# ActiveVisionLab/CrossScore

Measured on AMD Instinct MI355X. Metric: query-images/sec at 518x518, 5 ref views, bs=8; score-map MAE vs ref, higher is better.
Workload: dtype fp16

## Files before the change

### crossscore_amd/csrc/rowln.hip

```cpp
#include "cs_common.h"
#include <atomic>

namespace {

__device__ __forceinline__ float rl_add_other_half(float x) {
  const auto r = __builtin_amdgcn_permlane32_swap(__float_as_uint(x), __float_as_uint(x), false, false);
  return __uint_as_float(r[0]) + __uint_as_float(r[1]);
}

template <int C, bool BF, int G2>
__global__ __launch_bounds__(C / 96 * 64) void cs_rowln_kernel(CsRowLnParams p) {
  constexpr int NW = C / 96, NT = NW * 64;
  constexpr bool NEXT = G2 > 0;
  constexpr int BK = 64, NSL = C / BK;
  constexpr int APITCH = C * 2 + 16;
  constexpr int WPITCH = BK * 2 + 16;
  constexpr int WBUF = C * WPITCH;
  constexpr int ACH = C / 8, WCH = BK / 8;
  constexpr int AIT = 64 * ACH / NT, WIT = C * WCH / NT;
  static_assert(64 * ACH % NT == 0 && C * WCH % NT == 0, "staging maps");
  extern __shared__ __attribute__((aligned(16))) char smem[];
  char* As = smem;
  char* Ws = smem + 64 * APITCH;
  float* red = reinterpret_cast<float*>(Ws + 2 * WBUF);
  const int tid = threadIdx.x;
  const int lane = tid & 63;
  const int wv = __builtin_amdgcn_readfirstlane(tid >> 6);
  const int j = lane & 31, h = lane >> 5;
  const int row0 = blockIdx.x * 64;
  const int col0 = wv * 96;
  uint4 wreg[WIT];
#define RL_LOAD_W(REG, WP, LDW, SL)                                                                                \
  _Pragma("unroll") for (int it = 0; it < WIT; ++it) {                                                         \
    const int c_ = tid + it * NT, r_ = c_ / WCH, ch_ = c_ - r_ * WCH;                                          \
    REG[it] = *reinterpret_cast<const uint4*>((WP) + (size_t)r_ * (LDW) + (SL) * BK + ch_ * 8);                \
  }
#define RL_WRITE_W(REG, BUF)                                                                                   \
  _Pragma("unroll") for (int it = 0; it < WIT; ++it) {                                                         \
    const int c_ = tid + it * NT, r_ = c_ / WCH, ch_ = c_ - r_ * WCH;                                          \
    *reinterpret_cast<uint4*>(Ws + (BUF) * WBUF + r_ * WPITCH + ch_ * 16) = REG[it];                           \
  }
  RL_LOAD_W(wreg, p.W, p.ldw, 0)
  {
    uint4 areg[AIT];
#pragma unroll
    for (int it = 0; it < AIT; ++it) {
      const int c = tid + it * NT, r = c / ACH, ch = c - r * ACH;
      areg[it] = *reinterpret_cast<const uint4*>(p.A + (size_t)min(row0 + r, p.M - 1) * p.lda + ch * 8);
    }
#pragma unroll
    for (int it = 0; it < AIT; ++it) {
      const int c = tid + it * NT, r = c / ACH, ch = c - r * ACH;
      *reinterpret_cast<uint4*>(As + r * APITCH + ch * 16) = areg[it];
    }
  }
#define RL_KSLICE(SLICE)                                                                                       \
  _Pragma("unroll") for (int ks = 0; ks < BK / 16; ++ks) {                                                     \
    h16x8_t a[2], w[3];                                                                                        \
    _Pragma("unroll") for (int rb = 0; rb < 2; ++rb)                                                           \
      a[rb] = *reinterpret_cast<const h16x8_t*>(a_rd + rb * 32 * APITCH + ((SLICE) * (BK / 16) + ks) * 32);    \
    _Pragma("unroll") for (int ct = 0; ct < 3; ++ct) w[ct] = *reinterpret_cast<const h16x8_t*>(w_rd + ct * 32 * WPITCH + ks * 32); \
    _Pragma("unroll") for (int rb = 0; rb < 2; ++rb)                                                           \
      _Pragma("unroll") for (int ct = 0; ct < 3; ++ct) acc[rb][ct] = mfma_32x32x16<BF>(w[ct], a[rb], acc[rb][ct]); \
  }
  RL_WRITE_W(wreg, 0)
  __syncthreads();
  f32x16_t acc[2][3];
#pragma unroll
  for (int rb = 0; rb < 2; ++rb)
#pragma unroll
    for (int ct = 0; ct < 3; ++ct)
#pragma unroll
      for (int e = 0; e < 16; ++e) acc[rb][ct][e] = 0.f;
  const char* a_rd = As + j * APITCH + h * 16;
  for (int sl = 0; sl < NSL; ++sl) {
    if (sl + 1 < NSL) { RL_LOAD_W(wreg, p.W, p.ldw, sl + 1) }
    const char* w_rd = Ws + (sl & 1) * WBUF + (col0 + j) * WPITCH + h * 16;
    RL_KSLICE(sl)
    if (sl + 1 < NSL) { RL_WRITE_W(wreg, (sl + 1) & 1) }
    __syncthreads();
  }
  f32x4_t gam[3][4], bet[3][4];
#pragma unroll
  for (int ct = 0; ct < 3; ++ct)
#pragma unroll
    for (int g = 0; g < 4; ++g) {
      const int c = col0 + 32 * ct + 8 * g + 4 * h;
      const f32x4_t b4 = *reinterpret_cast<const f32x4_t*>(p.bias + c);
      gam[ct][g] = *reinterpret_cast<const f32x4_t*>(p.gamma + c);
      bet[ct][g] = *reinterpret_cast<const f32x4_t*>(p.beta + c);
#pragma unroll
      for (int rb = 0; rb < 2; ++rb)
#pragma unroll
        for (int i = 0; i < 4; ++i) acc[rb][ct][4 * g + i] += b4[i];
    }
  if (p.resid) {
#pragma unroll
    for (int rb = 0; rb < 2; ++rb) {
      const float* rr = p.resid + (size_t)min(row0 + 32 * rb + j, p.M - 1) * p.ldr + col0 + 4 * h;
#pragma unroll
      for (int ct = 0; ct < 3; ++ct)
#pragma unroll
        for (int g = 0; g < 4; ++g) {
          const f32x4_t r4 = *reinterpret_cast<const f32x4_t*>(rr + 32 * ct + 8 * g);
#pragma unroll
          for (int i = 0; i < 4; ++i) acc[rb][ct][4 * g + i] += r4[i];
        }
    }
  }
  float mean[2], rstd[2];
#pragma unroll
  for (int rb = 0; rb < 2; ++rb) {
    float s = 0.f;
#pragma unroll
    for (int ct = 0; ct < 3; ++ct)
#pragma unroll
      for (int e = 0; e < 16; e += 4) s += (acc[rb][ct][e] + acc[rb][ct][e + 1]) + (acc[rb][ct][e + 2] + acc[rb][ct][e + 3]);
    s = rl_add_other_half(s);
    if (h == 0) red[(0 * NW + wv) * 64 + 32 * rb + j] = s;
  }
  __syncthreads();
#pragma unroll
  for (int rb = 0; rb < 2; ++rb) {
    float s = 0.f;
#pragma unroll
    for (int w2 = 0; w2 < NW; ++w2) s += red[(0 * NW + w2) * 64 + 32 * rb + j];
    mean[rb] = s * (1.0f / C);
    float q = 0.f;
#pragma unroll
    for (int ct = 0; ct < 3; ++ct)
#pragma unroll
      for (int e = 0; e < 16; ++e) {
        const float d = acc[rb][ct][e] - mean[rb];
        q = fmaf(d, d, q);
      }
    q = rl_add_other_half(q);
    if (h == 0) red[(1 * NW + wv) * 64 + 32 * rb + j] = q;
  }
  __syncthreads();
#pragma unroll
  for (int rb = 0; rb < 2; ++rb) {
    float q = 0.f;
#pragma unroll
    for (int w2 = 0; w2 < NW; ++w2) q += red[(1 * NW + w2) * 64 + 32 * rb + j];
    rstd[rb] = 1.0f / sqrtf(q * (1.0f / C) + p.eps);
  }
#pragma unroll
  for (int rb = 0; rb < 2; ++rb) {
    const int row = row0 + 32 * rb + j;
    if (row < p.M) {
      float* o32 = p.out_f32 ? p.out_f32 + (size_t)row * C + col0 + 4 * h : nullptr;
      h16_t* o16 = p.out_f16 ? p.out_f16 + (size_t)row * C + col0 + 4 * h : nullptr;
#pragma unroll
      for (int ct = 0; ct < 3; ++ct)
#pragma unroll
        for (int g = 0; g < 4; ++g) {
          f32x4_t y;
#pragma unroll
          for (int i = 0; i < 4; ++i) y[i] = (acc[rb][ct][4 * g + i] - mean[rb]) * rstd[rb] * gam[ct][g][i] + bet[ct][g][i];
          if (o32) *reinterpret_cast<f32x4_t*>(o32 + 32 * ct + 8 * g) = y;
          if (o16) {
            uint2 o;
            o.x = pack_o16x2<BF>(y[0], y[1]);
            o.y = pack_o16x2<BF>(y[2], y[3]);
            *reinterpret_cast<uint2*>(o16 + 32 * ct + 8 * g) = o;
          }
        }
    }
  }
  if constexpr (NEXT) {
#pragma unroll
    for (int rb = 0; rb < 2; ++rb) {
      char* arow = As + (32 * rb + j) * APITCH + (col0 + 4 * h) * 2;
#pragma unroll
      for (int ct = 0; ct < 3; ++ct)
#pragma unroll
        for (int g = 0; g < 4; ++g) {
          float y[4];
#pragma unroll
          for (int i = 0; i < 4; ++i) y[i] = (acc[rb][ct][4 * g + i] - mean[rb]) * rstd[rb] * gam[ct][g][i] + bet[ct][g][i];
          uint2 o;
          o.x = pack_o16x2<BF>(y[0], y[1]);
          o.y = pack_o16x2<BF>(y[2], y[3]);
          *reinterpret_cast<uint2*>(arow + (32 * ct + 8 * g) * 2) = o;
        }
    }
    RL_LOAD_W(wreg, p.W2, p.ldw2, 0)
    RL_WRITE_W(wreg, 0)
    __syncthreads();
    constexpr int nsl2 = G2 * NSL;
#pragma unroll
    for (int s2 = 0; s2 < nsl2; ++s2) {
      const int grp = s2 / NSL, sl = s2 - grp * NSL;
      if (sl == 0) {
#pragma unroll
        for (int rb = 0; rb < 2; ++rb)
#pragma unroll
          for (int ct = 0; ct < 3; ++ct)
#pragma unroll
            for (int e = 0; e < 16; ++e) acc[rb][ct][e] = 0.f;
      }
      if (s2 + 1 < nsl2) {
        const int g2 = (s2 + 1) / NSL, sn = (s2 + 1) - g2 * NSL;
        RL_LOAD_W(wreg, p.W2 + (size_t)g2 * C * p.ldw2, p.ldw2, sn)
      }
      const char* w_rd = Ws + (s2 & 1) * WBUF + (col0 + j) * WPITCH + h * 16;
      RL_KSLICE(sl)
      if (s2 + 1 < nsl2) { RL_WRITE_W(wreg, (s2 + 1) & 1) }
      __syncthreads();
      if (sl == NSL - 1) {
#pragma unroll
        for (int rb = 0; rb < 2; ++rb) {
          const int row = row0 + 32 * rb + j;
          if (row < p.M) {
            h16_t* o2 = p.out2 + (size_t)row * p.ld2 + grp * C + col0 + 4 * h;
            const float* b2 = p.bias2 + grp * C + col0 + 4 * h;
#pragma unroll
            for (int ct = 0; ct < 3; ++ct)
#pragma unroll
              for (int g = 0; g < 4; ++g) {
                const f32x4_t b4 = *reinterpret_cast<const f32x4_t*>(b2 + 32 * ct + 8 * g);
                float v[4];
#pragma unroll
                for (int i = 0; i < 4; ++i) {
                  v[i] = acc[rb][ct][4 * g + i] + b4[i];
                  if (p.act2 == 1) v[i] = fmaxf(v[i], 0.f);
                  if (p.act2 == 2) v[i] = v[i] >= 0.f ? v[i] : 0.01f * v[i];
                }
                uint2 o;
                o.x = pack_o16x2<BF>(v[0], v[1]);
                o.y = pack_o16x2<BF>(v[2], v[3]);
                *reinterpret_cast<uint2*>(o2 + 32 * ct + 8 * g) = o;
              }
          }
        }
      }
    }
  }
#undef RL_KSLICE
#undef RL_LOAD_W
#undef RL_WRITE_W
}

}

extern "C" int cs_rowln_supported(int C) { return C == 384; }

extern "C" const char* cs_rowln_check(const CsRowLnParams* p, int C) {
  if (!cs_rowln_supported(C)) return "linear + LayerNorm: built for C = 384";
  if (!p->A || !p->W || !p->bias || !p->gamma || !p->beta || (!p->out_f32 && !p->out_f16 && !p->n2)) return "linear + LayerNorm: null operand";
  if (p->n2) {
    if ((p->n2 != C && p->n2 != 3 * C) || p->act2 < 0 || p->act2 > 2) return "linear + LayerNorm: the second stage takes C or 3 C output columns and act2 in 0..2";
    if (!p->W2 || !p->bias2 || !p->out2) return "linear + LayerNorm: null operand (second stage)";
    if (p->ldw2 % 8 || p->ldw2 < C || p->ld2 % 4 || p->ld2 < p->n2) return "linear + LayerNorm: row strides must keep 16-byte rows (second stage)";
    if (((uintptr_t)p->W2 | (uintptr_t)p->bias2) & 15 || ((uintptr_t)p->out2 & 7)) return "linear + LayerNorm: operands must be 16-byte aligned (second stage)";
  }
  if (p->M <= 0) return "linear + LayerNorm: empty shape";
  if (p->lda % 8 || p->ldw % 8 || p->lda < C || p->ldw < C || (p->resid && (p->ldr % 4 || p->ldr < C))) return "linear + LayerNorm: row strides must keep 16-byte rows";
  if (((uintptr_t)p->A | (uintptr_t)p->W | (uintptr_t)p->bias | (uintptr_t)p->gamma | (uintptr_t)p->beta | (uintptr_t)p->resid | (uintptr_t)p->out_f32 |
       (uintptr_t)p->out_f16) & 15)
    return "linear + LayerNorm: operands must be 16-byte aligned";
  return nullptr;
}

extern "C" hipError_t cs_rowln_launch(const CsRowLnParams* p, int C, int bf16, hipStream_t st) {
  if (C != 384) return hipErrorInvalidValue;
  constexpr int CC = 384, NW = CC / 96;
  constexpr int lds = 64 * (CC * 2 + 16) + 2 * CC * (64 * 2 + 16) + 2 * NW * 64 * 4;
  static std::atomic<bool> attr_done[16];
  int dev = 0;
  if (hipGetDevice(&dev) != hipSuccess || dev < 0 || dev >= 16) return hipErrorInvalidDevice;
  if (!attr_done[dev]) {
    const void* fns[6] = {reinterpret_cast<const void*>(cs_rowln_kernel<384, true, 0>), reinterpret_cast<const void*>(cs_rowln_kernel<384, false, 0>),
                          reinterpret_cast<const void*>(cs_rowln_kernel<384, true, 1>), reinterpret_cast<const void*>(cs_rowln_kernel<384, false, 1>),
                          reinterpret_cast<const void*>(cs_rowln_kernel<384, true, 3>), reinterpret_cast<const void*>(cs_rowln_kernel<384, false, 3>)};
    for (const void* f : fns)
      if (hipError_t e = hipFuncSetAttribute(f, hipFuncAttributeMaxDynamicSharedMemorySize, lds); e != hipSuccess) return e;
    attr_done[dev] = true;
  }
  const dim3 grid((p->M + 63) / 64), block(NW * 64);
#define RL_GO(G) do { if (bf16) hipLaunchKernelGGL((cs_rowln_kernel<384, true, G>), grid, block, lds, st, *p);  \
                      else hipLaunchKernelGGL((cs_rowln_kernel<384, false, G>), grid, block, lds, st, *p); } while (0)
  if (p->n2 == 0) RL_GO(0);
  else if (p->n2 == CC) RL_GO(1);
  else if (p->n2 == 3 * CC) RL_GO(3);
  else return hipErrorInvalidValue;
#undef RL_GO
  return hipGetLastError();
}
```

Before: 1409.

## Split row-LN GEMM across 8 waves with 16x16 MFMA and unified weight pipeline

Doubles the block to 8 waves, splitting the 64 rows into two 32-row halves so each wave computes a 32x96 tile with 16x16x32 MFMAs instead of 64x96 with 32x32x16. The first GEMM and the follow-on GEMM groups are merged into one unrolled slice loop with two register buffers prefetching weights two slices ahead, which removes the separate W2 prologue stall. LayerNorm reductions now use permlane16+permlane32 swaps. The aim is more latency hiding and occupancy, at the cost of extra LDS traffic per MFMA and a larger unrolled code body.

```diff
diff --git a/crossscore_amd/csrc/rowln.hip b/crossscore_amd/csrc/rowln.hip
--- a/crossscore_amd/csrc/rowln.hip
+++ b/crossscore_amd/csrc/rowln.hip
@@ -3,21 +3,29 @@
 
 namespace {
 
-__device__ __forceinline__ float rl_add_other_half(float x) {
+typedef unsigned u32x4_t __attribute__((ext_vector_type(4)));
+
+__device__ __forceinline__ float rl_add_lane16(float x) {
+  const auto r = __builtin_amdgcn_permlane16_swap(__float_as_uint(x), __float_as_uint(x), false, false);
+  return __uint_as_float(r[0]) + __uint_as_float(r[1]);
+}
+__device__ __forceinline__ float rl_add_lane32(float x) {
   const auto r = __builtin_amdgcn_permlane32_swap(__float_as_uint(x), __float_as_uint(x), false, false);
   return __uint_as_float(r[0]) + __uint_as_float(r[1]);
 }
 
 template <int C, bool BF, int G2>
-__global__ __launch_bounds__(C / 96 * 64) void cs_rowln_kernel(CsRowLnParams p) {
-  constexpr int NW = C / 96, NT = NW * 64;
+__global__ __launch_bounds__(C / 96 * 128) void cs_rowln_kernel(CsRowLnParams p) {
+  constexpr int NW = C / 96, NT = NW * 128;
   constexpr bool NEXT = G2 > 0;
   constexpr int BK = 64, NSL = C / BK;
+  constexpr int TOT = NSL * (1 + G2);
   constexpr int APITCH = C * 2 + 16;
   constexpr int WPITCH = BK * 2 + 16;
   constexpr int WBUF = C * WPITCH;
   constexpr int ACH = C / 8, WCH = BK / 8;
   constexpr int AIT = 64 * ACH / NT, WIT = C * WCH / NT;
+  constexpr int NCT = 6;
   static_assert(64 * ACH % NT == 0 && C * WCH % NT == 0, "staging maps");
   extern __shared__ __attribute__((aligned(16))) char smem[];
   char* As = smem;
@@ -26,212 +34,190 @@
   const int tid = threadIdx.x;
   const int lane = tid & 63;
   const int wv = __builtin_amdgcn_readfirstlane(tid >> 6);
-  const int j = lane & 31, h = lane >> 5;
+  const int rh = wv / NW, cg = wv - rh * NW;
+  const int fr = lane & 15, cq = lane >> 4;
   const int row0 = blockIdx.x * 64;
-  const int col0 = wv * 96;
-  uint4 wreg[WIT];
-#define RL_LOAD_W(REG, WP, LDW, SL)                                                                                \
-  _Pragma("unroll") for (int it = 0; it < WIT; ++it) {                                                         \
-    const int c_ = tid + it * NT, r_ = c_ / WCH, ch_ = c_ - r_ * WCH;                                          \
-    REG[it] = *reinterpret_cast<const uint4*>((WP) + (size_t)r_ * (LDW) + (SL) * BK + ch_ * 8);                \
+  const int rloc = 32 * rh + fr;
+  const int col0 = cg * 96;
+  u32x4_t wreg0[WIT], wreg1[WIT];
+#define RL_LOAD_W(REG, T)                                                                                      \
+  {                                                                                                            \
+    const h16_t* wp_ = (T) < NSL ? p.W : p.W2 + (size_t)(((T) - NSL) / NSL) * C * p.ldw2;                      \
+    const int ldw_ = (T) < NSL ? p.ldw : p.ldw2;                                                               \
+    _Pragma("unroll") for (int it = 0; it < WIT; ++it) {                                                       \
+      const int c_ = tid + it * NT, r_ = c_ / WCH, ch_ = c_ - r_ * WCH;                                        \
+      REG[it] = *reinterpret_cast<const u32x4_t*>(wp_ + (size_t)r_ * ldw_ + ((T) % NSL) * BK + ch_ * 8);   \
+    }                                                                                                          \
   }
 #define RL_WRITE_W(REG, BUF)                                                                                   \
   _Pragma("unroll") for (int it = 0; it < WIT; ++it) {                                                         \
     const int c_ = tid + it * NT, r_ = c_ / WCH, ch_ = c_ - r_ * WCH;                                          \
-    *reinterpret_cast<uint4*>(Ws + (BUF) * WBUF + r_ * WPITCH + ch_ * 16) = REG[it];                           \
-  }
-  RL_LOAD_W(wreg, p.W, p.ldw, 0)
+    *reinterpret_cast<u32x4_t*>(Ws + (BUF) * WBUF + r_ * WPITCH + ch_ * 16) = REG[it];                           \
+  }
+  RL_LOAD_W(wreg0, 0)
   {
-    uint4 areg[AIT];
+    u32x4_t areg[AIT];
 #pragma unroll
     for (int it = 0; it < AIT; ++it) {
       const int c = tid + it * NT, r = c / ACH, ch = c - r * ACH;
-      areg[it] = *reinterpret_cast<const uint4*>(p.A + (size_t)min(row0 + r, p.M - 1) * p.lda + ch * 8);
-    }
+      areg[it] = *reinterpret_cast<const u32x4_t*>(p.A + (size_t)min(row0 + r, p.M - 1) * p.lda + ch * 8);
+    }
+    RL_LOAD_W(wreg1, 1)
 #pragma unroll
     for (int it = 0; it < AIT; ++it) {
       const int c = tid + it * NT, r = c / ACH, ch = c - r * ACH;
-      *reinterpret_cast<uint4*>(As + r * APITCH + ch * 16) = areg[it];
-    }
-  }
-#define RL_KSLICE(SLICE)                                                                                       \
-  _Pragma("unroll") for (int ks = 0; ks < BK / 16; ++ks) {                                                     \
-    h16x8_t a[2], w[3];                                                                                        \
-    _Pragma("unroll") for (int rb = 0; rb < 2; ++rb)                                                           \
-      a[rb] = *reinterpret_cast<const h16x8_t*>(a_rd + rb * 32 * APITCH + ((SLICE) * (BK / 16) + ks) * 32);    \
-    _Pragma("unroll") for (int ct = 0; ct < 3; ++ct) w[ct] = *reinterpret_cast<const h16x8_t*>(w_rd + ct * 32 * WPITCH + ks * 32); \
-    _Pragma("unroll") for (int rb = 0; rb < 2; ++rb)                                                           \
-      _Pragma("unroll") for (int ct = 0; ct < 3; ++ct) acc[rb][ct] = mfma_32x32x16<BF>(w[ct], a[rb], acc[rb][ct]); \
-  }
-  RL_WRITE_W(wreg, 0)
+      *reinterpret_cast<u32x4_t*>(As + r * APITCH + ch * 16) = areg[it];
+    }
+  }
+#define RL_KSLICE(T)                                                                                           \
+  {                                                                                                            \
+    const char* w_rd = Ws + ((T) & 1) * WBUF + (col0 + fr) * WPITCH + cq * 16;                                 \
+    _Pragma("unroll") for (int ks = 0; ks < BK / 32; ++ks) {                                                   \
+      h16x8_t a[2], w[NCT];                                                                                    \
+      _Pragma("unroll") for (int rt = 0; rt < 2; ++rt)                                                         \
+        a[rt] = *reinterpret_cast<const h16x8_t*>(a_rd + rt * 16 * APITCH + (((T) % NSL) * (BK / 32) + ks) * 64); \
+      _Pragma("unroll") for (int ct = 0; ct < NCT; ++ct) w[ct] = *reinterpret_cast<const h16x8_t*>(w_rd + ct * 16 * WPITCH + ks * 64); \
+      _Pragma("unroll") for (int ct = 0; ct < NCT; ++ct)                                                       \
+        _Pragma("unroll") for (int rt = 0; rt < 2; ++rt) acc[rt][ct] = mfma_16x16x32<BF>(w[ct], a[rt], acc[rt][ct]); \
+    }                                                                                                          \
+  }
+  RL_WRITE_W(wreg0, 0)
   __syncthreads();
-  f32x16_t acc[2][3];
-#pragma unroll
-  for (int rb = 0; rb < 2; ++rb)
-#pragma unroll
-    for (int ct = 0; ct < 3; ++ct)
-#pragma unroll
-      for (int e = 0; e < 16; ++e) acc[rb][ct][e] = 0.f;
-  const char* a_rd = As + j * APITCH + h * 16;
-  for (int sl = 0; sl < NSL; ++sl) {
-    if (sl + 1 < NSL) { RL_LOAD_W(wreg, p.W, p.ldw, sl + 1) }
-    const char* w_rd = Ws + (sl & 1) * WBUF + (col0 + j) * WPITCH + h * 16;
-    RL_KSLICE(sl)
-    if (sl + 1 < NSL) { RL_WRITE_W(wreg, (sl + 1) & 1) }
+  f32x4_t acc[2][NCT];
+#pragma unroll
+  for (int rt = 0; rt < 2; ++rt)
+#pragma unroll
+    for (int ct = 0; ct < NCT; ++ct) acc[rt][ct] = f32x4_t{0.f, 0.f, 0.f, 0.f};
+  const char* a_rd = As + rloc * APITCH + cq * 16;
+#pragma unroll
+  for (int t = 0; t < TOT; ++t) {
+    if (t + 2 < TOT) {
+      if ((t & 1) == 0) { RL_LOAD_W(wreg0, t + 2) } else { RL_LOAD_W(wreg1, t + 2) }
+      __builtin_amdgcn_sched_barrier(0);
+    }
+    if (NEXT && t >= NSL && t % NSL == 0) {
+#pragma unroll
+      for (int rt = 0; rt < 2; ++rt)
+#pragma unroll
+        for (int ct = 0; ct < NCT; ++ct) acc[rt][ct] = f32x4_t{0.f, 0.f, 0.f, 0.f};
+    }
+    RL_KSLICE(t)
+    if (t + 1 < TOT) {
+      if ((t & 1) == 0) { RL_WRITE_W(wreg1, 1) } else { RL_WRITE_W(wreg0, 0) }
+    }
     __syncthreads();
-  }
-  f32x4_t gam[3][4], bet[3][4];
-#pragma unroll
-  for (int ct = 0; ct < 3; ++ct)
-#pragma unroll
-    for (int g = 0; g < 4; ++g) {
-      const int c = col0 + 32 * ct + 8 * g + 4 * h;
-      const f32x4_t b4 = *reinterpret_cast<const f32x4_t*>(p.bias + c);
-      gam[ct][g] = *reinterpret_cast<const f32x4_t*>(p.gamma + c);
-      bet[ct][g] = *reinterpret_cast<const f32x4_t*>(p.beta + c);
-#pragma unroll
-      for (int rb = 0; rb < 2; ++rb)
-#pragma unroll
-        for (int i = 0; i < 4; ++i) acc[rb][ct][4 * g + i] += b4[i];
-    }
-  if (p.resid) {
-#pragma unroll
-    for (int rb = 0; rb < 2; ++rb) {
-      const float* rr = p.resid + (size_t)min(row0 + 32 * rb + j, p.M - 1) * p.ldr + col0 + 4 * h;
-#pragma unroll
-      for (int ct = 0; ct < 3; ++ct)
-#pragma unroll
-        for (int g = 0; g < 4; ++g) {
-          const f32x4_t r4 = *reinterpret_cast<const f32x4_t*>(rr + 32 * ct + 8 * g);
-#pragma unroll
-          for (int i = 0; i < 4; ++i) acc[rb][ct][4 * g + i] += r4[i];
-        }
-    }
-  }
-  float mean[2], rstd[2];
-#pragma unroll
-  for (int rb = 0; rb < 2; ++rb) {
-    float s = 0.f;
-#pragma unroll
-    for (int ct = 0; ct < 3; ++ct)
-#pragma unroll
-      for (int e = 0; e < 16; e += 4) s += (acc[rb][ct][e] + acc[rb][ct][e + 1]) + (acc[rb][ct][e + 2] + acc[rb][ct][e + 3]);
-    s = rl_add_other_half(s);
-    if (h == 0) red[(0 * NW + wv) * 64 + 32 * rb + j] = s;
-  }
-  __syncthreads();
-#pragma unroll
-  for (int rb = 0; rb < 2; ++rb) {
-    float s = 0.f;
-#pragma unroll
-    for (int w2 = 0; w2 < NW; ++w2) s += red[(0 * NW + w2) * 64 + 32 * rb + j];
-    mean[rb] = s * (1.0f / C);
-    float q = 0.f;
-#pragma unroll
-    for (int ct = 0; ct < 3; ++ct)
-#pragma unroll
-      for (int e = 0; e < 16; ++e) {
-        const float d = acc[rb][ct][e] - mean[rb];
-        q = fmaf(d, d, q);
-      }
-    q = rl_add_other_half(q);
-    if (h == 0) red[(1 * NW + wv) * 64 + 32 * rb + j] = q;
-  }
-  __syncthreads();
-#pragma unroll
-  for (int rb = 0; rb < 2; ++rb) {
-    float q = 0.f;
-#pragma unroll
-    for (int w2 = 0; w2 < NW; ++w2) q += red[(1 * NW + w2) * 64 + 32 * rb + j];
-    rstd[rb] = 1.0f / sqrtf(q * (1.0f / C) + p.eps);
-  }
-#pragma unroll
-  for (int rb = 0; rb < 2; ++rb) {
-    const int row = row0 + 32 * rb + j;
-    if (row < p.M) {
-      float* o32 = p.out_f32 ? p.out_f32 + (size_t)row * C + col0 + 4 * h : nullptr;
-      h16_t* o16 = p.out_f16 ? p.out_f16 + (size_t)row * C + col0 + 4 * h : nullptr;
-#pragma unroll
-      for (int ct = 0; ct < 3; ++ct)
-#pragma unroll
-        for (int g = 0; g < 4; ++g) {
-          f32x4_t y;
-#pragma unroll
-          for (int i = 0; i < 4; ++i) y[i] = (acc[rb][ct][4 * g + i] - mean[rb]) * rstd[rb] * gam[ct][g][i] + bet[ct][g][i];
-          if (o32) *reinterpret_cast<f32x4_t*>(o32 + 32 * ct + 8 * g) = y;
-          if (o16) {
+    if (t == NSL - 1) {
+      float mean[2], rstd[2];
+      f32x4_t gam[NCT], bet[NCT];
+#pragma unroll
+      for (int ct = 0; ct < NCT; ++ct) {
+        const int c = col0 + 16 * ct + 4 * cq;
+        const f32x4_t b4 = *reinterpret_cast<const f32x4_t*>(p.bias + c);
+        gam[ct] = *reinterpret_cast<const f32x4_t*>(p.gamma + c);
+        bet[ct] = *reinterpret_cast<const f32x4_t*>(p.beta + c);
+#pragma unroll
+        for (int rt = 0; rt < 2; ++rt) acc[rt][ct] += b4;
+      }
+      if (p.resid) {
+        f32x4_t r4[2][NCT];
+#pragma unroll
+        for (int rt = 0; rt < 2; ++rt) {
+          const float* rr = p.resid + (size_t)min(row0 + rloc + 16 * rt, p.M - 1) * p.ldr + col0 + 4 * cq;
+#pragma unroll
+          for (int ct = 0; ct < NCT; ++ct) r4[rt][ct] = *reinterpret_cast<const f32x4_t*>(rr + 16 * ct);
+        }
+        __builtin_amdgcn_sched_barrier(0);
+#pragma unroll
+        for (int rt = 0; rt < 2; ++rt)
+#pragma unroll
+          for (int ct = 0; ct < NCT; ++ct) acc[rt][ct] += r4[rt][ct];
+      }
+#pragma unroll
+      for (int rt = 0; rt < 2; ++rt) {
+        float s = 0.f;
+#pragma unroll
+        for (int ct = 0; ct < NCT; ++ct) s += (acc[rt][ct][0] + acc[rt][ct][1]) + (acc[rt][ct][2] + acc[rt][ct][3]);
+        s = rl_add_lane32(rl_add_lane16(s));
+        if (cq == 0) red[(0 * NW + cg) * 64 + rloc + 16 * rt] = s;
+      }
+      __syncthreads();
+#pragma unroll
+      for (int rt = 0; rt < 2; ++rt) {
+        float s = 0.f;
+#pragma unroll
+        for (int w2 = 0; w2 < NW; ++w2) s += red[(0 * NW + w2) * 64 + rloc + 16 * rt];
+        mean[rt] = s * (1.0f / C);
+        float q = 0.f;
+#pragma unroll
+        for (int ct = 0; ct < NCT; ++ct)
+#pragma unroll
+          for (int e = 0; e < 4; ++e) {
+            const float d = acc[rt][ct][e] - mean[rt];
+            q = fmaf(d, d, q);
+          }
+        q = rl_add_lane32(rl_add_lane16(q));
+        if (cq == 0) red[(1 * NW + cg) * 64 + rloc + 16 * rt] = q;
+      }
+      __syncthreads();
+#pragma unroll
+      for (int rt = 0; rt < 2; ++rt) {
+        float q = 0.f;
+#pragma unroll
+        for (int w2 = 0; w2 < NW; ++w2) q += red[(1 * NW + w2) * 64 + rloc + 16 * rt];
+        rstd[rt] = 1.0f / sqrtf(q * (1.0f / C) + p.eps);
+      }
+#pragma unroll
+      for (int rt = 0; rt < 2; ++rt) {
+        const int row = row0 + rloc + 16 * rt;
+        f32x4_t y[NCT];
+#pragma unroll
+        for (int ct = 0; ct < NCT; ++ct)
+#pragma unroll
+          for (int i = 0; i < 4; ++i) y[ct][i] = (acc[rt][ct][i] - mean[rt]) * rstd[rt] * gam[ct][i] + bet[ct][i];
+        uint2 y16[NCT];
+#pragma unroll
+        for (int ct = 0; ct < NCT; ++ct) y16[ct] = make_uint2(pack_o16x2<BF>(y[ct][0], y[ct][1]), pack_o16x2<BF>(y[ct][2], y[ct][3]));
+        if (row < p.M) {
+          const size_t o = (size_t)row * C + col0 + 4 * cq;
+          if (p.out_f32) {
+#pragma unroll
+            for (int ct = 0; ct < NCT; ++ct) *reinterpret_cast<f32x4_t*>(p.out_f32 + o + 16 * ct) = y[ct];
+          }
+          if (p.out_f16) {
+#pragma unroll
+            for (int ct = 0; ct < NCT; ++ct) *reinterpret_cast<uint2*>(p.out_f16 + o + 16 * ct) = y16[ct];
+          }
+        }
+        if constexpr (NEXT) {
+          char* arow = As + (rloc + 16 * rt) * APITCH + (col0 + 4 * cq) * 2;
+#pragma unroll
+          for (int ct = 0; ct < NCT; ++ct) *reinterpret_cast<uint2*>(arow + 16 * ct * 2) = y16[ct];
+        }
+      }
+      if constexpr (NEXT) __syncthreads();
+    }
+    if (NEXT && t >= NSL && t % NSL == NSL - 1) {
+      const int grp = (t - NSL) / NSL;
+#pragma unroll
+      for (int rt = 0; rt < 2; ++rt) {
+        const int row = row0 + rloc + 16 * rt;
+        if (row < p.M) {
+          h16_t* o2 = p.out2 + (size_t)row * p.ld2 + grp * C + col0 + 4 * cq;
+          const float* b2 = p.bias2 + grp * C + col0 + 4 * cq;
+#pragma unroll
+          for (int ct = 0; ct < NCT; ++ct) {
+            const f32x4_t b4 = *reinterpret_cast<const f32x4_t*>(b2 + 16 * ct);
+            float v[4];
+#pragma unroll
+            for (int i = 0; i < 4; ++i) {
+              v[i] = acc[rt][ct][i] + b4[i];
+              if (p.act2 == 1) v[i] = fmaxf(v[i], 0.f);
+              if (p.act2 == 2) v[i] = v[i] >= 0.f ? v[i] : 0.01f * v[i];
+            }
             uint2 o;
-            o.x = pack_o16x2<BF>(y[0], y[1]);
-            o.y = pack_o16x2<BF>(y[2], y[3]);
-            *reinterpret_cast<uint2*>(o16 + 32 * ct + 8 * g) = o;
-          }
-        }
-    }
-  }
-  if constexpr (NEXT) {
-#pragma unroll
-    for (int rb = 0; rb < 2; ++rb) {
-      char* arow = As + (32 * rb + j) * APITCH + (col0 + 4 * h) * 2;
-#pragma unroll
-      for (int ct = 0; ct < 3; ++ct)
-#pragma unroll
-        for (int g = 0; g < 4; ++g) {
-          float y[4];
-#pragma unroll
-          for (int i = 0; i < 4; ++i) y[i] = (acc[rb][ct][4 * g + i] - mean[rb]) * rstd[rb] * gam[ct][g][i] + bet[ct][g][i];
-          uint2 o;
-          o.x = pack_o16x2<BF>(y[0], y[1]);
-          o.y = pack_o16x2<BF>(y[2], y[3]);
-          *reinterpret_cast<uint2*>(arow + (32 * ct + 8 * g) * 2) = o;
-        }
-    }
-    RL_LOAD_W(wreg, p.W2, p.ldw2, 0)
-    RL_WRITE_W(wreg, 0)
-    __syncthreads();
-    constexpr int nsl2 = G2 * NSL;
-#pragma unroll
-    for (int s2 = 0; s2 < nsl2; ++s2) {
-      const int grp = s2 / NSL, sl = s2 - grp * NSL;
-      if (sl == 0) {
-#pragma unroll
-        for (int rb = 0; rb < 2; ++rb)
-#pragma unroll
-          for (int ct = 0; ct < 3; ++ct)
-#pragma unroll
-            for (int e = 0; e < 16; ++e) acc[rb][ct][e] = 0.f;
-      }
-      if (s2 + 1 < nsl2) {
-        const int g2 = (s2 + 1) / NSL, sn = (s2 + 1) - g2 * NSL;
-        RL_LOAD_W(wreg, p.W2 + (size_t)g2 * C * p.ldw2, p.ldw2, sn)
-      }
-      const char* w_rd = Ws + (s2 & 1) * WBUF + (col0 + j) * WPITCH + h * 16;
-      RL_KSLICE(sl)
-      if (s2 + 1 < nsl2) { RL_WRITE_W(wreg, (s2 + 1) & 1) }
-      __syncthreads();
-      if (sl == NSL - 1) {
-#pragma unroll
-        for (int rb = 0; rb < 2; ++rb) {
-          const int row = row0 + 32 * rb + j;
-          if (row < p.M) {
-            h16_t* o2 = p.out2 + (size_t)row * p.ld2 + grp * C + col0 + 4 * h;
-            const float* b2 = p.bias2 + grp * C + col0 + 4 * h;
-#pragma unroll
-            for (int ct = 0; ct < 3; ++ct)
-#pragma unroll
-              for (int g = 0; g < 4; ++g) {
-                const f32x4_t b4 = *reinterpret_cast<const f32x4_t*>(b2 + 32 * ct + 8 * g);
-                float v[4];
-#pragma unroll
-                for (int i = 0; i < 4; ++i) {
-                  v[i] = acc[rb][ct][4 * g + i] + b4[i];
-                  if (p.act2 == 1) v[i] = fmaxf(v[i], 0.f);
-                  if (p.act2 == 2) v[i] = v[i] >= 0.f ? v[i] : 0.01f * v[i];
-                }
-                uint2 o;
-                o.x = pack_o16x2<BF>(v[0], v[1]);
-                o.y = pack_o16x2<BF>(v[2], v[3]);
-                *reinterpret_cast<uint2*>(o2 + 32 * ct + 8 * g) = o;
-              }
+            o.x = pack_o16x2<BF>(v[0], v[1]);
+            o.y = pack_o16x2<BF>(v[2], v[3]);
+            *reinterpret_cast<uint2*>(o2 + 16 * ct) = o;
           }
         }
       }
@@ -278,7 +264,7 @@
       if (hipError_t e = hipFuncSetAttribute(f, hipFuncAttributeMaxDynamicSharedMemorySize, lds); e != hipSuccess) return e;
     attr_done[dev] = true;
   }
-  const dim3 grid((p->M + 63) / 64), block(NW * 64);
+  const dim3 grid((p->M + 63) / 64), block(NW * 128);
 #define RL_GO(G) do { if (bf16) hipLaunchKernelGGL((cs_rowln_kernel<384, true, G>), grid, block, lds, st, *p);  \
                       else hipLaunchKernelGGL((cs_rowln_kernel<384, false, G>), grid, block, lds, st, *p); } while (0)
   if (p->n2 == 0) RL_GO(0);
```

After: 1417, median of 6. No clear change (+0.6%).
